# esq4/nind-denoise

Measured on AMD Instinct MI355X. Metric: megapixels/sec denoised, UtNet cs=256 on 24 MP frames, 1/2/4/8 MI355X, higher is better.
Workload: dtype f32; 1 GPU; configs[1]: one 6000x4000 (24.0 MP) fp32 frame per step, f32 storage in the conv stack (fp32 accumulate), UtNet(funit=64,PReLU) random-init (seed 123), cs=264 (nearest valid to the named size; the reference rejects 256 / 512) ucs=200 ol=64 -> 1276 tiles/frame, tiles per conv-stack launch 256, crop->infer->stitch device resident (frame and canvas in HBM); every tile's input is the whole cs x cs cro; tiles_per_frame=1276, parallelism=single GPU

## Files before the change

include/nind_hip.h:

```cpp
#ifndef NIND_HIP_H
#define NIND_HIP_H

#include <stddef.h>
#include <stdint.h>

#ifdef __cplusplus
extern "C" {
#endif

typedef enum nd_status {
    ND_OK = 0,
    ND_EINVAL = -1,
    ND_ENOMEM = -2,
    ND_EHIP = -3
} nd_status;

typedef enum nd_act {
    ND_ACT_NONE = 0,
    ND_ACT_PRELU = 1,
    ND_ACT_ELU = 2,
    ND_ACT_HARDSWISH = 3
} nd_act;

typedef enum nd_layer_kind {
    ND_CONV3 = 0,
    ND_CONVT3 = 1,
    ND_CONVT2S2 = 2,
    ND_CONV1 = 3,
    ND_CONV2S2 = 4
} nd_layer_kind;

typedef enum nd_dtype {
    ND_F32 = 0,
    ND_BF16 = 1,
    ND_F16 = 2
} nd_dtype;

typedef enum nd_flags {
    ND_FLAG_NO_SPLITK = 1,
    ND_FLAG_DIRECT_CONV = 2,
    ND_FLAG_W1D_REGS = 4,
    ND_FLAG_UNFUSED_POOL = 16,
    ND_FLAG_TILE_ENCODER = 32,
    ND_FLAG_TILE_LEVEL2 = 64,
    ND_FLAG_FIND_NOISE = 128,
    ND_FLAG_TILE_SKIPS = 256,
    ND_FLAG_TILE_WINO = 512,
    ND_FLAG_FULL_TILES = 8
} nd_flags;

int nd_version(void);
const char *nd_last_error(void);

int nd_tile_grid(int width, int height, int cs, int ucs, int ol, int *cols, int *rows, int *pad);
int nd_tile_geom(int i, int width, int height, int cs, int ucs, int ol,
                 int *x0, int *y0, int usefuldim[4], int usefulstart[2]);

int nd_tile_gather(const float *img_chw, int width, int height, int cs, int ucs, int ol,
                   int tile_begin, int tile_count, float *tiles_nchw, void *stream);
int nd_stitch_add(float *canvas_chw, int width, int height, int cs, int ucs, int ol,
                  const float *tiles_nchw, int tile_begin, int tile_count, void *stream);

int nd_utnet_num_tensors(void);
const char *nd_utnet_tensor_name(int idx);
size_t nd_utnet_packed_bytes(int funit, int dtype);
int nd_utnet_pack_weights(int funit, int dtype, const float *const *tensors, int n_tensors,
                          void *packed_host, size_t packed_bytes);

int nd_utnet_pack_weights_device(int funit, int dtype, const float *const *dev_tensors, int n_tensors, void *packed_dev,
                                 size_t packed_bytes, void *stream);
// ... 91 lines not shown
                               void *const *bucket_events, int n_events);
int nd_utnet_grad_buckets(int funit, size_t *offsets, size_t *counts, int max);
int nd_adam_step(float *params, const float *grads, float *m, float *v, float *vmax, size_t n, float lr, float beta1,
                 float beta2, float eps, int step, int amsgrad, void *stream);

size_t nd_ssim_workspace_bytes(int n, int c, int h, int w);
int nd_ssim(const float *x, const float *y, int n, int c, int h, int w, float *out, void *workspace, size_t workspace_bytes,
            void *stream);
int nd_ms_ssim(const float *x, const float *y, int n, int c, int h, int w, float *out, void *workspace,
               size_t workspace_bytes, void *stream);
int nd_mse(const float *x, const float *y, size_t count, float *out, void *workspace, size_t workspace_bytes, void *stream);

size_t nd_ssim_loss_workspace_bytes(int n, int c, int h, int w);
int nd_ssim_loss_grad(const float *x, const float *y, int n, int c, int h, int w, int multiscale, float weight,
                      float *loss_acc, float *gx, int accumulate, void *workspace, size_t workspace_bytes, void *stream);

size_t nd_ssim_padded_workspace_bytes(int n, int c, int h, int w, int window);
int nd_ssim_padded(const float *x, const float *y, int n, int c, int h, int w, int window, float *out, void *workspace,
                   size_t workspace_bytes, void *stream);
int nd_ssim_padded_grad(const float *x, const float *y, int n, int c, int h, int w, int window, const float *gout, float *gx,
                        void *workspace, size_t workspace_bytes, void *stream);

int nd_wino_mosaic(int p, int B, int *bx, int *by, long *tiles, long *tiles_per_image);

size_t nd_winograd_packed_bytes(int tile, int cin, int cout);
int nd_winograd_pack(int tile, int kind, int cin, int cout, const float *w, const float *bias, void *packed,
                     size_t packed_bytes);
size_t nd_layer_winograd_workspace_bytes(int tile, int kind, int batch, int cin, int cout, int h, int w);
int nd_layer_forward_winograd(int tile, int kind, int act, float slope, const void *packed, const float *x, int batch,
                              int cin, int h, int w, int cout, float *y, void *workspace, size_t workspace_bytes, int flags,
                              void *stream);

int nd_conv_bench(int kind, int dtype, int batch, int cin, int cout, int h, int w, int variant, int iters,
                  void *workspace, size_t workspace_bytes, void *stream, float *mean_ms);

int nd_winograd_bench(int tile, int kind, int batch, int cin, int cout, int h, int w, int iters, void *workspace,
                      size_t workspace_bytes, void *stream, float *mean_ms);
int nd_winograd_bench_flags(int tile, int kind, int batch, int cin, int cout, int h, int w, int iters, int flags, void *workspace,
                            size_t workspace_bytes, void *stream, float *mean_ms);

int nd_num_conv_variants(void);
const char *nd_conv_variant_name(int variant);

#ifdef __cplusplus
}
#endif
// ... 2 lines not shown
```

nind_denoise_amd/_lib.py:

```python
import ctypes
import os
from ctypes import POINTER, c_char_p, c_double, c_float, c_int, c_long, c_size_t, c_void_p

_HERE = os.path.dirname(os.path.abspath(__file__))
LIB_PATH = os.path.join(_HERE, "libnind_hip.so")

ND_F32, ND_BF16, ND_F16 = 0, 1, 2
DTYPE = {"f32": 0, "fp32": 0, "float32": 0, "bf16": 1, "bfloat16": 1, "f16": 2, "fp16": 2, "float16": 2}
ACT = {"none": 0, "PReLU": 1, "ELU": 2, "Hardswish": 3}
KIND = {"conv3": 0, "convT3": 1, "convT2s2": 2, "conv1": 3, "conv2s2": 4}
FLAG_NO_SPLITK, FLAG_DIRECT_CONV, FLAG_W1D_REGS, FLAG_FULL_TILES, FLAG_UNFUSED_POOL, FLAG_TILE_ENCODER, FLAG_TILE_LEVEL2 = 1, 2, 4, 8, 16, 32, 64
FLAG_FIND_NOISE = 128
FLAG_TILE_SKIPS = 256
FLAG_TILE_WINO = 512
PROGRESS_FN = ctypes.CFUNCTYPE(None, c_void_p, c_int, c_int, c_int)


class StepProfile(ctypes.Structure):
    _fields_ = [("ms", c_float), ("ms_xform_in", c_float), ("ms_gemm", c_float), ("ms_xform_out", c_float),
                ("form", c_int), ("kind", c_int), ("flops", c_double), ("mfma_flops", c_double), ("bytes", c_double),
                ("xform_bytes_in", c_double), ("xform_bytes_out", c_double)]


FORM_NAMES = {-1: "pool", 0: "direct", 1: "w1d_f43", 2: "w1d_f23", 3: "wino3p_f6x6"}


class NindHipError(RuntimeError):
    pass


class NindHipMissing(ImportError):
    pass


_lib = None

# ... 55 lines not shown
    "nd_utnet_train_workspace_bytes_hw": (c_size_t, [c_int] * 4),
    "nd_utnet_train_workspace_init_hw": (c_int, [c_void_p, c_size_t, c_int, c_int, c_int, c_int, c_void_p]),
    "nd_utnet_train_forward_hw": (c_int, [c_int, c_int, c_int, c_void_p, c_void_p, c_void_p, c_void_p, c_int, c_int, c_int, c_void_p,
                                          c_size_t, c_void_p]),
    "nd_utnet_train_backward_hw": (c_int, [c_int, c_int, c_int, c_void_p, c_void_p, c_void_p, c_void_p, c_void_p, c_int, c_int, c_int,
                                           c_void_p, c_size_t, c_void_p, POINTER(c_void_p), c_int]),
    "nd_utnet_train_step_hw": (c_int, [c_int, c_int, c_void_p, c_void_p, c_void_p, c_void_p, c_void_p, c_void_p, c_float, c_float,
                                       c_float, c_float, c_void_p, c_int, c_int, c_int, c_int, c_void_p, c_size_t, c_void_p,
                                       POINTER(c_void_p), c_int]),
    "nd_adam_step": (c_int, [c_void_p] * 5 + [c_size_t, c_float, c_float, c_float, c_float, c_int, c_int, c_void_p]),
    "nd_ssim_workspace_bytes": (c_size_t, [c_int] * 4),
    "nd_ssim": (c_int, [c_void_p, c_void_p] + [c_int] * 4 + [c_void_p, c_void_p, c_size_t, c_void_p]),
    "nd_ms_ssim": (c_int, [c_void_p, c_void_p] + [c_int] * 4 + [c_void_p, c_void_p, c_size_t, c_void_p]),
    "nd_ssim_loss_workspace_bytes": (c_size_t, [c_int] * 4),
    "nd_ssim_loss_grad": (c_int, [c_void_p, c_void_p] + [c_int] * 5 + [c_float, c_void_p, c_void_p, c_int, c_void_p, c_size_t,
                                  c_void_p]),
    "nd_ssim_padded_workspace_bytes": (c_size_t, [c_int] * 5),
    "nd_ssim_padded": (c_int, [c_void_p, c_void_p] + [c_int] * 5 + [c_void_p, c_void_p, c_size_t, c_void_p]),
    "nd_ssim_padded_grad": (c_int, [c_void_p, c_void_p] + [c_int] * 5 + [c_void_p, c_void_p, c_void_p, c_size_t, c_void_p]),
    "nd_mse": (c_int, [c_void_p, c_void_p, c_size_t, c_void_p, c_void_p, c_size_t, c_void_p]),
    "nd_conv_bench": (c_int, [c_int] * 9 + [c_void_p, c_size_t, c_void_p, POINTER(c_float)]),
    "nd_winograd_bench": (c_int, [c_int] * 8 + [c_void_p, c_size_t, c_void_p, POINTER(c_float)]),
    "nd_winograd_bench_flags": (c_int, [c_int] * 9 + [c_void_p, c_size_t, c_void_p, POINTER(c_float)]),
    "nd_wino_mosaic": (c_int, [c_int, c_int, POINTER(c_int), POINTER(c_int), POINTER(c_long), POINTER(c_long)]),
    "nd_num_conv_variants": (c_int, []),
    "nd_conv_variant_name": (c_char_p, [c_int]),
}

EXPORTS = tuple(_SIGNATURES)


def load():
    global _lib
    if _lib is not None:
        return _lib
    if not os.path.isfile(LIB_PATH):
        raise NindHipMissing(
            f"{LIB_PATH} not found: build it with `make -C nind_denoise_amd/csrc` (or __graft_entry__.build()). "
            "nind_denoise_amd has no CPU fallback for the denoise hot path.")
    import torch
    lib = ctypes.CDLL(LIB_PATH)
    for name, (res, args) in _SIGNATURES.items():
        fn = getattr(lib, name)
        fn.restype = res
        fn.argtypes = args
    _lib = lib
# ... 39 lines not shown
```

nind_denoise_amd/csrc/nd_common.h:

```cpp
#pragma once
#include <hip/hip_runtime.h>

#include <stdarg.h>
#include <stdint.h>
#include <stdio.h>

#include "nind_hip.h"

void nd_set_error(const char *fmt, ...);
#define ND_FAIL(code, ...)        \
    do {                          \
        nd_set_error(__VA_ARGS__); \
        return (code);            \
    } while (0)
#define ND_HIP(call)                                                                         \
    do {                                                                                     \
        hipError_t e_ = (call);                                                              \
        if (e_ != hipSuccess) ND_FAIL(ND_EHIP, "%s failed: %s", #call, hipGetErrorString(e_)); \
    } while (0)
#define ND_TRY(call)        \
    do {                    \
        int r_ = (call);    \
        if (r_ != 0) return r_; \
    } while (0)
// ... 9 lines not shown
    long np() const { return pstride; }
    long used() const { return (long)B * Hb * Wb; }
};

struct ConvDesc {
    int kind = ND_CONV3;
    int act = ND_ACT_NONE;
    float slope = 1.f;
    const float *slope_dev = nullptr;
    const float *wpk = nullptr;
    const float *bias = nullptr;
    int cin = 0, cout = 0;
    QpBuf in = {};
    QpBuf out = {};
    int out_plane0 = 0;
    int variant = -1;
    int in_plane0 = 0;
    float *pre = nullptr;
    long pre_plane = 0;
    float *part = nullptr;
    size_t part_bytes = 0;
    bool nosplit = false;
    bool tile_wino = false;
    int nbatch = 1;
    long in_bs = 0, out_bs = 0;
    size_t w_bs = 0;
    const QpBuf *pool = nullptr;
    int roi_r0 = 0, roi_c0 = 0, roi_rows = 0, roi_cols = 0;
    QpBuf in2 = {};
    int in2_plane0 = 0, in2_from = 0;
    const int *in2_origin = nullptr;
    long in2_origin_max = 0;
    int w_kb = 0, w_kb0 = 0;
    QpBuf add = {};
    int add_plane0 = 0;
    const int *add_origin = nullptr;
    long add_origin_max = 0;
};
int nd_check_in2(const char *who, const ConvDesc &d, int KB, long reach);
int nd_check_add(const char *who, const ConvDesc &d, long reach);
static const size_t kSplitScratchBytes = (size_t)512 * 64 * 1024 * 4;
int nd_launch_conv(const ConvDesc &d, hipStream_t stream);
bool nd_conv_pool_fits(const ConvDesc &d);
bool nd_conv_roi_fits(const ConvDesc &d);
int nd_conv_variant_count();
int nd_conv_variant_gemm(int cin, int cout);
// ... 2 lines not shown
size_t nd_wino_scratch_bytes(int T, const QpBuf &in, int cin, int cout);
int nd_launch_conv_wino(int T, const ConvDesc &d, void *scratch, size_t scratch_bytes, hipStream_t s, hipEvent_t *ev2 = nullptr);
long nd_wino_launch_tiles(int T, const ConvDesc &d);
void nd_wino_xform_bytes(int T, const QpBuf &in, int cin, int cout, long tiles, double *bytes_in, double *bytes_out);
size_t nd_w1d_packed_floats(int T, int cin, int cout);
int nd_w1d_pack(int T, int kind, int cin, int cout, const float *w, const float *bias, float *packed);
bool nd_w1d_fits(int T, const QpBuf &in);
int nd_launch_conv_w1d(int T, const ConvDesc &d, hipStream_t stream);
bool nd_w2d_ok(const QpBuf &in);
long nd_w2d_tiles(const QpBuf &in, int cout);
int nd_launch_conv_w2d(const ConvDesc &d, hipStream_t stream);
bool nd_f43_w2d(const QpBuf &in, int cout, bool pre, int flags);
int nd_launch_conv_f43(const ConvDesc &d, int flags, hipStream_t stream);
static inline size_t nd_buf_slack(int Wb) { return (size_t)10 * Wb + 8 + 2048; }
int nd_device(int *dev, int *ncus = nullptr);
int nd_raise_lds(int dev, const void *fn, size_t bytes);
int nd_once_per_device(int dev, int (*init)());
int nd_check_in_planes(const char *who, const ConvDesc &d, int KB, bool takes_in2 = false, bool takes_add = false);
int nd_check_out(const char *who, const ConvDesc &d, int oh, int ow, bool at_least);
int nd_check_int32(const char *who, const QpBuf &in);
int nd_check_roi(const char *who, const ConvDesc &d, int Hv, int Wv, bool refused, const char *why);
static inline int nd_check_flags(int flags, bool frame_loop = false, bool unet_frame = false) {
    const int known = ND_FLAG_NO_SPLITK | ND_FLAG_DIRECT_CONV | ND_FLAG_W1D_REGS | ND_FLAG_FULL_TILES | ND_FLAG_UNFUSED_POOL |
                      ND_FLAG_TILE_ENCODER | ND_FLAG_TILE_WINO | (frame_loop ? ND_FLAG_TILE_LEVEL2 | ND_FLAG_TILE_SKIPS : 0) | (unet_frame ? ND_FLAG_FIND_NOISE : 0);
    if (flags & ~known) ND_FAIL(ND_EINVAL, "unknown flag bits 0x%x", flags);
    return ND_OK;
}
const char *nd_conv_variant_label(int v);

static inline int nd_mtiles(int kind, int cout) {
    return kind == ND_CONVT2S2 ? (4 * cout + 255) / 256 * 8 : (cout + 127) / 128 * 4;
}
struct NdUpRow { int a, b, co; };
__host__ __device__ static inline NdUpRow nd_up_row(int m, int cout, int dt) {
    NdUpRow r;
    const int cpp = dt == ND_F32 ? 4 : 8, q = cout / cpp;
    const int G = m / (2 * cpp), e = m % cpp;
    r.b = (m / cpp) & 1;
    r.a = G / q;
    r.co = cpp * (G % q) + e;
    return r;
}
static inline int nd_taps(int kind) { return (kind == ND_CONV3 || kind == ND_CONVT3) ? 9 : (kind == ND_CONV2S2 ? 4 : 1); }
static inline int nd_kblocks(int cin, int dt = ND_F32) { return (cin + 2 * nd_cpp(dt) - 1) / (2 * nd_cpp(dt)); }
static inline size_t nd_bias_offset(int kind, int cin, int cout, int dt = ND_F32, int w1d_T = 0) {
    return (size_t)nd_mtiles(kind, cout) * nd_kblocks(cin, dt) * (w1d_T ? 3 * (w1d_T + 2) : nd_taps(kind)) * 256;
}
// ... 37 lines not shown
```

nind_denoise_amd/csrc/pack.hip:

```cpp
#include <string.h>

#include "nd_common.h"

static thread_local char g_err[512] = "";

void nd_set_error(const char *fmt, ...) {
    va_list ap;
    va_start(ap, fmt);
    vsnprintf(g_err, sizeof(g_err), fmt, ap);
    va_end(ap);
}

extern "C" const char *nd_last_error(void) { return g_err; }
extern "C" int nd_version(void) { return 112; }

static inline uint16_t f32_to_bf16_rne(float f) {
    uint32_t u;
    memcpy(&u, &f, 4);
    if ((u & 0x7fffffffu) > 0x7f800000u) return (uint16_t)((u >> 16) | 0x40);
    return (uint16_t)((u + 0x7fffu + ((u >> 16) & 1u)) >> 16);
}
static inline uint16_t f32_to_f16_rne(float f) {
    const _Float16 h = (_Float16)f;
    uint16_t u;
    memcpy(&u, &h, 2);
    return u;
}

void nd_pack_layer(int kind, int cin, int cout, int dt, const float *w, const float *bias, float *packed) {
    const int taps = nd_taps(kind);
    const int KB = nd_kblocks(cin, dt);
    const int MT = nd_mtiles(kind, cout);
    const int M = kind == ND_CONVT2S2 ? 4 * cout : cout;
    const int cpp = nd_cpp(dt);
    float *bp = packed + nd_bias_offset(kind, cin, cout, dt);
    auto weff = [&](int m, int ci, int t) -> float {
        if (m >= M || ci >= cin) return 0.f;
// ... 51 lines not shown
```

nind_denoise_amd/csrc/utnet.hip:

```cpp
#include <string.h>

#include <string>
#include <vector>

#include "nd_common.h"

#include "utnet_net.h"

extern "C" int nd_utnet_num_tensors(void) { return (int)tensor_names().size(); }
extern "C" const char *nd_utnet_tensor_name(int idx) {
    const auto &n = tensor_names();
    return (idx >= 0 && idx < (int)n.size()) ? n[idx].c_str() : nullptr;
}

extern "C" size_t nd_utnet_packed_bytes(int funit, int dtype) {
    if (check_funit(funit, dtype) != ND_OK) return 0;
    return blob_layout(funit, dtype).total * sizeof(float);
}

extern "C" int nd_utnet_pack_weights(int funit, int dtype, const float *const *tensors, int n_tensors, void *packed_host,
                                     size_t packed_bytes) {
    ND_TRY(check_funit(funit, dtype));
    if (n_tensors != nd_utnet_num_tensors()) ND_FAIL(ND_EINVAL, "nd_utnet_pack_weights: expected %d tensors, got %d", nd_utnet_num_tensors(), n_tensors);
    const BlobLayout bl = blob_layout(funit, dtype);
// ... 627 lines not shown
    d.part_bytes = kSplitScratchBytes;
    return d;
}
int launch_form(const LayerForm &fm, const ConvDesc &d, void *scratch, size_t scratch_bytes, hipStream_t s) {
    switch (fm.fam) {
        case LF_W1D: return nd_launch_conv_w1d(fm.T, d, s);
        case LF_W2D: return nd_launch_conv_w2d(d, s);
        case LF_WINO3P: return nd_launch_conv_wino(fm.T, d, scratch, scratch_bytes, s);
        default: return nd_launch_conv(d, s);
    }
}

int layer_forward(const LayerForm &fm, int kind, int act, float slope, int dt, const void *packed, const float *x, int batch,
                  int cin, int h, int w, int cout, float *y, void *ws, size_t ws_bytes, int variant, int flags, hipStream_t s) {
    const LayerPlan pl = layer_plan(kind, batch, cin, cout, h, w, (char *)ws, dt);
    ND_HIP(hipMemsetAsync(ws, 0, pl.bytes, s));
    ND_TRY(nd_launch_nchw_to_qp(x, cin, pl.in, 0, s));
    ConvDesc d = layer_desc(fm, kind, cin, cout, dt, (const float *)packed, pl);
    d.act = act;
    d.slope = slope;
    d.variant = variant;
    d.nosplit = (flags & ND_FLAG_NO_SPLITK) != 0;
    d.tile_wino = (flags & ND_FLAG_TILE_WINO) != 0;
    ND_TRY(launch_form(fm, d, (char *)ws + pl.bytes, ws_bytes - pl.bytes, s));
    return nd_launch_qp_to_nchw(pl.out, 0, y, cout, s);
}
}

extern "C" size_t nd_layer_workspace_bytes(int kind, int batch, int cin, int cout, int h, int w, int dtype) {
    if (dtype < ND_F32 || dtype > ND_F16 || kind < 0 || kind > 4 || batch <= 0 || cin <= 0 || cout <= 0 || h <= 0 || w <= 0) return 0;
    if (kind == ND_CONV3 && (h < 3 || w < 3)) return 0;
    return layer_plan(kind, batch, cin, cout, h, w, nullptr, dtype).bytes;
}

extern "C" int nd_layer_forward(int kind, int act, float slope, int dtype, const void *packed, const float *x, int batch,
                                int cin, int h, int w, int cout, float *y, void *ws, size_t ws_bytes, int variant, int flags,
                                void *stream) {
    ND_TRY(nd_check_flags(flags));
    if (dtype < ND_F32 || dtype > ND_F16) ND_FAIL(ND_EINVAL, "nd_layer_forward: unsupported dtype %d", dtype);
    const size_t need = nd_layer_workspace_bytes(kind, batch, cin, cout, h, w, dtype);
    if (!need) ND_FAIL(ND_EINVAL, "nd_layer_forward: bad shape");
    if (!ws || ws_bytes < need) ND_FAIL(ND_ENOMEM, "nd_layer_forward: workspace %zu B given, %zu B needed", ws_bytes, need);
    if (cout % nd_cpp(dtype)) ND_FAIL(ND_EINVAL, "nd_layer_forward: cout must be a multiple of %d", nd_cpp(dtype));
    return layer_forward(kDirect, kind, act, slope, dtype, packed, x, batch, cin, h, w, cout, y, ws, ws_bytes, variant, flags,
                         (hipStream_t)stream);
}
// ... 133 lines not shown

extern "C" int nd_winograd_bench(int tile, int kind, int batch, int cin, int cout, int h, int w, int iters, void *ws,
                                 size_t ws_bytes, void *stream, float *mean_ms) {
    return nd_winograd_bench_flags(tile, kind, batch, cin, cout, h, w, iters, 0, ws, ws_bytes, stream, mean_ms);
}
extern "C" int nd_winograd_bench_flags(int tile, int kind, int batch, int cin, int cout, int h, int w, int iters, int flags, void *ws,
                                       size_t ws_bytes, void *stream, float *mean_ms) {
    ND_TRY(nd_check_flags(flags));
    const size_t need = nd_layer_winograd_workspace_bytes(tile, kind, batch, cin, cout, h, w);
    if (!need) ND_FAIL(ND_EINVAL, "nd_winograd_bench: bad shape / kind / tile");
    const LayerForm fm = wino_form(tile);
    const size_t wfloats = wino_packed_floats(fm, cin, cout);
    const size_t total = ((need + 255) & ~(size_t)255) + wfloats * 4;
    if (!ws || ws_bytes < total) ND_FAIL(ND_ENOMEM, "nd_winograd_bench: workspace %zu B given, %zu B needed", ws_bytes, total);
    hipStream_t s = (hipStream_t)stream;
    LayerPlan pl = layer_plan(kind, batch, cin, cout, h, w, (char *)ws, ND_F32);
    float *wpk = (float *)((char *)ws + ((need + 255) & ~(size_t)255));
    fill_random(ws, pl.bytes, wpk, wfloats, ND_F32, kind, cin, cout, s);
    ConvDesc d = layer_desc(fm, kind, cin, cout, ND_F32, wpk, pl);
    d.act = ND_ACT_PRELU;
    d.slope = 0.2f;
    d.nosplit = (flags & ND_FLAG_NO_SPLITK) != 0;
    d.tile_wino = (flags & ND_FLAG_TILE_WINO) != 0;
    return time_form("nd_winograd_bench", fm, d, (char *)ws + pl.bytes, need - pl.bytes, iters, s, mean_ms);
}
```

nind_denoise_amd/csrc/utnet_net.h:

```cpp
#pragma once
#include <string.h>

#include <string>
#include <vector>

#include "nd_common.h"

namespace {

struct LayerSpec {
    const char *key;
    int kind;
    int cin_mul, cout_mul;
    int prelu;
};

const LayerSpec kLayers[] = {
    {"convs1.0", ND_CONV3, 0, 1, 0},    {"convs1.2", ND_CONV3, 1, 1, 1},    {"convs2.0", ND_CONV3, 1, 2, 2},
    {"convs2.2", ND_CONV3, 2, 2, 3},    {"convs3.0", ND_CONV3, 2, 4, 4},    {"convs3.2", ND_CONV3, 4, 4, 5},
    {"convs4.0", ND_CONV3, 4, 8, 6},    {"convs4.2", ND_CONV3, 8, 8, 7},    {"bottom.0", ND_CONV3, 8, 16, 8},
    {"bottom.2", ND_CONVT3, 16, 16, 9}, {"up1", ND_CONVT2S2, 16, 8, -1},    {"tconvs1.0", ND_CONVT3, 16, 8, 10},
    {"tconvs1.2", ND_CONVT3, 8, 8, 11}, {"up2", ND_CONVT2S2, 8, 4, -1},     {"tconvs2.0", ND_CONVT3, 8, 4, 12},
    {"tconvs2.2", ND_CONVT3, 4, 4, 13}, {"up3", ND_CONVT2S2, 4, 2, -1},     {"tconvs3.0", ND_CONVT3, 4, 2, 14},
    {"tconvs3.2", ND_CONVT3, 2, 2, 15}, {"up4", ND_CONVT2S2, 2, 1, -1},     {"tconvs4.0", ND_CONVT3, 2, 1, 16},
// ... 350 lines not shown
        }
        const LayerSpec &l = kLayers[st.layer];
        ConvDesc d;
        d.kind = l.kind;
        d.act = l.prelu >= 0 ? act : ND_ACT_NONE;
        d.slope = 0.25f;
        d.slope_dev = (l.prelu >= 0 && act == ND_ACT_PRELU) ? blob + l.prelu : nullptr;
        if (pre && l.prelu >= 0) {
            d.pre = pre[l.prelu].base;
            d.pre_plane = pre[l.prelu].np();
        }
        const int cin = lcin(l, f);
        d.cin = cin;
        d.cout = lcout(l, f);
        d.wpk = blob + bl.off[st.layer];
        d.bias = d.wpk + nd_bias_offset(l.kind, d.cin, d.cout, dt);
        d.in = pl.buf[st.src];
        d.out = pl.buf[st.dst];
        d.out_plane0 = st.dst_plane0_mul * f / cpp;
        d.part = pl.split;
        d.part_bytes = kSplitScratchBytes;
        d.nosplit = (flags & ND_FLAG_NO_SPLITK) != 0;
        d.tile_wino = (flags & ND_FLAG_TILE_WINO) != 0;
        const Form form = step_form(st, f, dt, flags, pl, bl, o.train_w1);
        if (o.rois && o.rois[this_step].rows > 0) {
            d.roi_r0 = o.rois[this_step].r0;
            d.roi_c0 = o.rois[this_step].c0;
            d.roi_rows = o.rois[this_step].rows;
            d.roi_cols = o.rois[this_step].cols;
        }
        for (int i = 0; i < o.nsrc2; ++i)
            if (o.src2[i].step == k && o.src2[i].addend) {
                d.add = o.src2[i].buf;
                d.add_plane0 = o.src2[i].plane0;
                d.add_origin = o.src2[i].origin;
                d.add_origin_max = o.src2[i].origin_max;
                d.w_kb = nd_kblocks(cin, dt);
                d.cin = o.src2[i].from * cpp;
            } else if (o.src2[i].step == k) {
                d.in2 = o.src2[i].buf;
                d.in2_plane0 = o.src2[i].plane0;
                d.in2_from = o.src2[i].from;
                d.in2_origin = o.src2[i].origin;
                d.in2_origin_max = o.src2[i].origin_max;
            }
        const bool next_is_pool = this_step + 1 < step_end && kSteps[this_step + 1].layer < 0;
// ... 251 lines not shown
    fp->bytes += fp->fold_wino_bytes;
}
inline int launch_skip_fold(int f, int flags, const float *blob, const BlobLayout &bl, int step, Form form, const QpBuf &cat, int planes,
                            const Roi &roi, int tstep, int nrows, int cols, float *split, char *wino, size_t wino_bytes, hipStream_t s) {
    const LayerSpec &l = kLayers[kSteps[step].layer];
    const int cin = lcin(l, f);
    ConvDesc d;
    d.kind = l.kind;
    d.act = ND_ACT_NONE;
    d.cin = planes * 4;
    d.cout = lcout(l, f);
    d.wpk = blob + bl.w1off[kSteps[step].layer];
    d.bias = d.wpk + nd_bias_offset(l.kind, cin, d.cout, ND_F32, kW1dTile);
    d.w_kb = nd_kblocks(cin);
    d.w_kb0 = planes / 2;
    d.in = cat;
    d.in_plane0 = planes;
    d.out = cat;
    d.out.pad = 1;
    d.out_plane0 = 0;
    d.part = split;
    d.part_bytes = split ? kSplitScratchBytes : 0;
    d.nosplit = (flags & ND_FLAG_NO_SPLITK) != 0;
    d.roi_r0 = roi.r0;
    d.roi_c0 = roi.c0;
    d.roi_rows = (nrows - 1) * tstep + roi.rows;
    d.roi_cols = (cols - 1) * tstep + roi.cols;
    if (form != FORM_WINO3P) return nd_launch_conv_w2d(d, s);
    d.wpk = blob + bl.woff[kSteps[step].layer];
    d.bias = nullptr;
    const int r_end = d.roi_r0 + d.roi_rows;
    for (int r0 = d.roi_r0; r0 < r_end; r0 += kFoldRows) {
        ConvDesc c = d;
        const int rows = r_end - r0 < kFoldRows ? r_end - r0 : kFoldRows;
        c.in.base = c.out.base = cat.base + (size_t)r0 * cat.Wb * 4;
        c.in.Hb = c.out.Hb = rows + 2;
        c.roi_r0 = 0;
        c.roi_rows = rows;
        ND_TRY(nd_launch_conv_wino(kWinoTile, c, wino, wino_bytes, s));
    }
    return ND_OK;
}

int frame_plan(int f, int dt, int flags, int W, int H, int cs, int ucs, int ol, int batch, FramePlan *fp) {
    *fp = FramePlan();
    ND_TRY(check_funit(f, dt));
// ... 63 lines not shown
```

nind_denoise_amd/csrc/winograd.hip:

```cpp
#include <stdlib.h>

#include <algorithm>
#include <atomic>
#include <thread>
#include <vector>

#include "nd_common.h"

typedef float f32x4 __attribute__((ext_vector_type(4)));

namespace {

__device__ __forceinline__ void tile_pos(long t, int TX, int TY, int &tx, int &ty, int &b) {
    const unsigned u = (unsigned)t, row = u / (unsigned)TX;
    tx = (int)(u - row * (unsigned)TX);
    b = (int)(row / (unsigned)TY);
    ty = (int)(row - (unsigned)b * (unsigned)TY);
}

template <int T> struct Wino;
template <> struct Wino<2> {
    static constexpr int A = 4;
    template <typename V> __host__ __device__ static void bt(const V *d, V *o) {
        o[0] = d[0] - d[2];
// ... 235 lines not shown
            for (int i = 0; i < A; ++i) d[i] = (okj && T * ty + i < Hb) ? src[(long)i * rs] : zero;
            Wino<T>::bt(d, o);
#pragma unroll
            for (int i = 0; i < A; ++i) sm[tl * RS + i * A + j] = o[i];
            }
        }
    }
    __syncthreads();
    {
        const int i = threadIdx.x / NTL, tl = threadIdx.x % NTL;
        const long t = t0 + tl;
        if (t < tiles) {
            f32x4 r[A], o[A];
#pragma unroll
            for (int j = 0; j < A; ++j) r[j] = sm[tl * RS + i * A + j];
            Wino<T>::bt(r, o);
            f32x4 *dst = v + (long)q * vnp + t;
#pragma unroll
            for (int j = 0; j < A; ++j) dst[(long)(i * A + j) * vbs] = o[j];
        }
    }
}

template <int T, int NTL, bool ADD = false, bool MOSAIC = false>
__global__ __launch_bounds__(NTL * (T + 2)) void k_wino_out2(const f32x4 *__restrict__ m, long mnp, long mbs, int B, int TY, int TX, int Hv,
                                                             int Wv, const float *__restrict__ bias, int act, float slope_imm,
                                                             const float *__restrict__ slope_dev, f32x4 *__restrict__ out, long onp,
                                                             int out_plane0, long out_img_stride, int Wo, int opad, f32x4 *__restrict__ pool, long pnp,
                                                             int Hp, int Wp, int ppad, const f32x4 *__restrict__ add = nullptr, long add_np = 0,
                                                             const int *__restrict__ origin_add = nullptr, int W_add = 0, int mp = 0,
                                                             int mbx = 0, int mby = 0) {
    static_assert(!(MOSAIC && ADD), "the mosaic form has no addend");
    constexpr int A = Wino<T>::A, RS = T * A + 1, NTH = NTL * A;
    __shared__ f32x4 sr[NTL * RS];
    __shared__ f32x4 so[T][NTL * T];
    const long tiles = MOSAIC ? (long)TY * TX : (long)B * TY * TX;
    const long t0 = (long)blockIdx.x * NTL;
    const int q = blockIdx.y;
    const f32x4 bv = ADD ? f32x4{0.f, 0.f, 0.f, 0.f} : *(const f32x4 *)(bias + 4 * q);
    const float slope = act == ND_ACT_NONE ? 1.f : (slope_dev ? *slope_dev : slope_imm);
    auto activate = [&](f32x4 y) {
#pragma unroll
        for (int e = 0; e < 4; ++e) {
            const float u = y[e];
            switch (act) {
                case ND_ACT_ELU: y[e] = u > 0.f ? u : expm1f(u); break;
// ... 87 lines not shown
    g.vnp = g.mnp = g.tiles;
    const long slack = 4096;
    g.vbs = (long)(2 * nd_kblocks(cin)) * g.vnp + slack;
    g.mbs = (long)((cout + 3) / 4) * g.mnp + slack;
    g.v_bytes = (size_t)positions(T) * g.vbs * 16;
    g.m_bytes = (size_t)positions(T) * g.mbs * 16;
}
WinoGeo wino_geo(int T, const QpBuf &in, int cin, int cout, int roi_rows = 0, int roi_cols = 0) {
    WinoGeo g;
    g.Hv = roi_rows > 0 ? roi_rows : in.Hb - 2;
    g.Wv = roi_rows > 0 ? roi_cols : in.Wb - 2;
    g.TY = (g.Hv + T - 1) / T;
    g.TX = (g.Wv + T - 1) / T;
    g.tiles = (long)in.B * g.TY * g.TX;
    wino_strides(T, cin, cout, g);
    return g;
}
bool wino_mosaic_rule(int T, const ConvDesc &d, int *bx, int *by, long *tiles) {
    if (T != 6 || d.kind != ND_CONVT3 || d.tile_wino || d.nosplit || d.roi_rows > 0 || d.pool || d.in2.base || d.add.base || d.pre) return false;
    if (d.in.Hb != d.in.Wb) return false;
    if (d.in.pad != 2) return false;
    long per_image;
    return nd_wino_mosaic(d.in.Hb - 2, d.in.B, bx, by, tiles, &per_image) == 1;
}
WinoGeo wino_geo_launch(int T, const ConvDesc &d) {
    WinoGeo g = wino_geo(T, d.in, d.cin, d.cout, d.roi_rows, d.roi_cols);
    int bx, by;
    long tiles;
    if (!wino_mosaic_rule(T, d, &bx, &by, &tiles)) return g;
    g.mp = g.Hv;
    g.mbx = bx;
    g.mby = by;
    g.TY = (by * g.mp + T - 1) / T;
    g.TX = (bx * g.mp + T - 1) / T;
    g.tiles = tiles;
    wino_strides(T, d.cin, d.cout, g);
    return g;
}
}

size_t nd_wino_packed_floats(int T, int cin, int cout) {
    return (size_t)positions(T) * gemm_floats(cin, cout) + (size_t)(cout + 3) / 4 * 4;
}

int nd_wino_pack(int T, int kind, int cin, int cout, const float *w, const float *bias, float *packed) {
    if (T != 2 && T != 4 && T != 6) ND_FAIL(ND_EINVAL, "winograd: tile must be 2, 4 or 6");
// ... 18 lines not shown
                    g[ky][kx] = kind == ND_CONV3 ? w[(((size_t)co * cin + ci) * 3 + ky) * 3 + kx]
                                                 : w[(((size_t)ci * cout + co) * 3 + (2 - ky)) * 3 + (2 - kx)];
            for (int kx = 0; kx < 3; ++kx) {
                double c[3] = {g[0][kx], g[1][kx], g[2][kx]}, o[8];
                if (T == 2) Wino<2>::g(c, o); else if (T == 4) Wino<4>::g(c, o); else Wino<6>::g(c, o);
                for (int i = 0; i < A; ++i) tmp[i][kx] = o[i];
            }
            for (int i = 0; i < A; ++i) {
                double o[8];
                if (T == 2) Wino<2>::g(tmp[i], o); else if (T == 4) Wino<4>::g(tmp[i], o); else Wino<6>::g(tmp[i], o);
                for (int j = 0; j < A; ++j) U[i][j] = o[j];
            }
            for (int i = 0; i < A; ++i)
                for (int j = 0; j < A; ++j) u[((size_t)(i * A + j) * cout + co) * cin + ci] = (float)U[i][j];
        }
    });
    const size_t gf = gemm_floats(cin, cout);
    parallel_for(P, [&](int p) { nd_pack_layer(ND_CONV1, cin, cout, ND_F32, u.data() + (size_t)p * cout * cin, nullptr, packed + p * gf); });
    float *b = packed + (size_t)P * gf;
    for (int co = 0; co < (cout + 3) / 4 * 4; ++co) b[co] = (bias && co < cout) ? bias[co] : 0.f;
    return ND_OK;
}

extern "C" int nd_wino_mosaic(int p, int B, int *bx, int *by, long *tiles, long *tiles_per_image) {
    if (p <= 0 || B <= 0 || !bx || !by || !tiles || !tiles_per_image) ND_FAIL(ND_EINVAL, "nd_wino_mosaic: bad arguments");
    const long T = 6, per = (long)B * ((p + T - 1) / T) * ((p + T - 1) / T);
    *tiles_per_image = *tiles = per;
    *bx = *by = 0;
    if (p < 8 || B < 2) return 0;
    auto count = [&](int x) { return (((long)x * p + T - 1) / T) * (((long)((B + x - 1) / x) * p + T - 1) / T); };
    long fewest = count(1);
    for (int x = 2; x <= B; ++x) fewest = std::min(fewest, count(x));
    long best = -1;
    int best_x = 0, best_y = 0, best_skew = 0;
    for (int x = B; x >= 1; --x) {
        const int y = (B + x - 1) / x, skew = x > y ? x - y : y - x;
        const long n = count(x);
        if (n * 100 > fewest * 101) continue;
        if (best < 0 || skew < best_skew || (skew == best_skew && n < best)) {
            best = n;
            best_x = x;
            best_y = y;
            best_skew = skew;
        }
    }
    if (best * 10 > per * 9) return 0;
// ... 37 lines not shown
    const bool src2 = d.in2.base != nullptr;
    if (src2) {
        if (T != 6) ND_FAIL(ND_EINVAL, "winograd: only the F(6x6) form has a second input source");
        ND_TRY(nd_check_in2("winograd", d, nd_kblocks(d.cin), (long)(d.roi_r0 + g.Hv + 1) * d.in2.Wb + d.roi_c0 + g.Wv + 2));
    }
    if (add) ND_TRY(nd_check_add("winograd", d, (long)(d.roi_r0 + g.Hv - 1 + d.add.pad) * d.add.Wb + d.roi_c0 + g.Wv - 1 + d.add.pad + 1));
    ND_TRY(nd_check_out("winograd", d, d.in.Hb - 2, d.in.Wb - 2, false));
    const long roi_in = roi ? (long)d.roi_r0 * d.in.Wb + d.roi_c0 : 0, roi_out = roi ? (long)d.roi_r0 * d.out.Wb + d.roi_c0 : 0;
    const int vHb = g.Hv + 2, vWb = g.Wv + 2;
    const size_t need = nd_wino_scratch_bytes(T, d.in, d.cin, d.cout);
    if (!scratch || scratch_bytes < need) ND_FAIL(ND_ENOMEM, "winograd: scratch %zu B given, %zu B needed", scratch_bytes, need);
    if (mosaic) {
        const size_t mneed = ((g.v_bytes + 255) & ~(size_t)255) + ((g.m_bytes + 255) & ~(size_t)255);
        if (g.mp < 8 || g.mp != d.in.Wb - 2 || (long)g.mbx * g.mby < d.in.B || (long)g.TY * g.TX != g.tiles || mneed > need)
            ND_FAIL(ND_EINVAL, "winograd: mosaic %d x %d at pitch %d does not fit %d images / the scratch bound", g.mbx, g.mby, g.mp, d.in.B);
    }
    if (g.tiles >= (1L << 31)) ND_FAIL(ND_EINVAL, "winograd: %ld tiles exceed the 32-bit tile index", g.tiles);
    const int P = positions(T);
    f32x4 *v = (f32x4 *)scratch;
    f32x4 *m = (f32x4 *)((char *)scratch + ((g.v_bytes + 255) & ~(size_t)255));
    const int in_planes = 2 * nd_kblocks(d.cin), out_planes = d.cout / 4;
    const f32x4 *x = (const f32x4 *)d.in.base + (long)d.in_plane0 * d.in.np() + roi_in;
    dim3 gi((unsigned)((g.tiles + 255) / 256), in_planes);
    constexpr int kNtl = 16;
    dim3 gi2((unsigned)((g.tiles + kNtl - 1) / kNtl), in_planes);
    if (T == 2)
        hipLaunchKernelGGL(k_wino_input<2>, gi, dim3(256), 0, s, x, d.in.np(), d.in.Hb, d.in.Wb, d.in.B, g.TY, g.TX, v, g.vnp, g.vbs);
    else if (mosaic)
        hipLaunchKernelGGL((k_wino_in2<6, kNtl, true>), gi2, dim3(kNtl * 8), 0, s, x, d.in.np(), vHb, vWb, (long)d.in.Hb * d.in.Wb, d.in.Wb, d.in.B, g.TY, g.TX, v, g.vnp,
                           g.vbs, nullptr, 0L, 0, nullptr, in_planes, g.mp, g.mbx, g.mby);
    else if (T == 6)
        hipLaunchKernelGGL((k_wino_in2<6, kNtl>), gi2, dim3(kNtl * 8), 0, s, x, d.in.np(), vHb, vWb, (long)d.in.Hb * d.in.Wb, d.in.Wb, d.in.B, g.TY, g.TX, v, g.vnp, g.vbs,
                           src2 ? (const f32x4 *)d.in2.base + (long)d.in2_plane0 * d.in2.np() + (roi ? (long)d.roi_r0 * d.in2.Wb + d.roi_c0 : 0) : nullptr,
                           d.in2.np(), d.in2.Wb, d.in2_origin, src2 ? d.in2_from : in_planes);
    else
        hipLaunchKernelGGL(k_wino_input<4>, gi, dim3(256), 0, s, x, d.in.np(), d.in.Hb, d.in.Wb, d.in.B, g.TY, g.TX, v, g.vnp, g.vbs);
    ND_HIP(hipGetLastError());
    if (ev2) ND_HIP(hipEventRecord(ev2[0], s));

    ConvDesc e;
    e.kind = ND_CONV1;
    e.cin = d.cin;
    e.cout = d.cout;
    e.wpk = d.wpk;
    e.bias = d.wpk + nd_bias_offset(ND_CONV1, cin_w, d.cout);
    e.w_kb = d.w_kb;
    e.w_kb0 = d.w_kb0;
    e.in = {(float *)v, in_planes, gB, g.TY, g.TX, 0, g.vnp, ND_F32};
    e.out = {(float *)m, out_planes, gB, g.TY, g.TX, 0, g.mnp, ND_F32};
// ... 58 lines not shown
```

nind_denoise_amd/networks/UtNet.py:

```python
import ctypes

import torch
from torch import nn

from .. import _lib
from ..synth import utnet_layer_table, utnet_prelu_keys

_ACTIVATIONS = {"PReLU": nn.PReLU, "ELU": nn.ELU, "Hardswish": nn.Hardswish}
_SHORT_DTYPE = {_lib.ND_F32: "f32", _lib.ND_BF16: "bf16", _lib.ND_F16: "f16"}


def canonical_compute_dtype(name):
    if name not in _lib.DTYPE:
        raise ValueError(f"unknown compute dtype {name!r}; choose one of {', '.join(_lib.DTYPE)}")
    return _SHORT_DTYPE[_lib.DTYPE[name]]


def valid_cs(cs):
    return cs >= 104 and (cs - 56) % 16 == 0


def nearest_valid_cs(cs):
    k = (cs - 56 + 8) // 16
    return max(104, 16 * k + 56)
# ... 61 lines not shown
        if st.generation != ctx.generation:
            raise RuntimeError("UtNet backward: another forward of this module ran under autograd since this graph was built; its "
                               "activations are gone (one forward/backward in flight per module -- as the reference's training loop runs)")
        batch, h, w = ctx.geom
        want_dx, want_p = ctx.needs_input_grad[2], ctx.needs_input_grad[3:]
        gy = gy.to(torch.float32).contiguous()
        dx = torch.empty(batch, 3, h, w, dtype=torch.float32, device=gy.device) if want_dx else None
        with torch.cuda.device(gy.device):
            _lib.check(_lib.load().nd_utnet_train_backward_hw(model.funit, _lib.ACT[model.activation], model.flags,
                                                              st.flat.data_ptr(), st.grads.data_ptr() if any(want_p) else None,
                                                              st.blobs.data_ptr(), gy.data_ptr(), dx.data_ptr() if want_dx else None,
                                                              batch, h, w, st.ws.data_ptr(), st.ws.numel(), _lib.stream_ptr(gy.device),
                                                              None, 0), "nd_utnet_train_backward_hw")
        grads = []
        for n, shape, want in zip(ctx.names, ctx.shapes, want_p):
            off, cnt = st.ranges[n]
            grads.append(st.grads[off:off + cnt].view(shape).clone() if want else None)
        return (None, None, dx) + tuple(grads)


class UtNet(nn.Module):
    split_k = True
    mosaic_wino = True
    winograd = True
    w1d_regs = False
    useful_only = True
    fused_pool = True
    share_encoder = True
    share_level2 = True
    fold_skips = True

    def __init__(self, funit=64, activation='PReLU', compute_dtype='f32'):
        super().__init__()
        funit = int(funit)
        compute_dtype = canonical_compute_dtype(compute_dtype)
        if activation not in _ACTIVATIONS:
            exit(f'UtNet: unknown activation function: {activation}')
        self.funit, self.activation = funit, activation
        groups = {}
        for key, kind, cin, cout, k in utnet_layer_table(funit):
            if kind == "conv":
                layer = nn.Conv2d(cin, cout, k)
            elif kind == "convT":
                layer = nn.ConvTranspose2d(cin, cout, k)
            else:
                layer = nn.ConvTranspose2d(cin, cout, k, stride=2)
# ... 11 lines not shown
        for name in order:
            g = groups[name]
            self.add_module(name, nn.Sequential(*[g[i] for i in sorted(g)]) if isinstance(g, dict) else g)
        self._packed = {}
        self.pack_on_device = True
        self._workspaces = {}
        self.max_cached_workspaces = 2
        self.compute_dtype = compute_dtype
        self.weights_generation = 0

    def set_compute_dtype(self, name):
        self.compute_dtype = canonical_compute_dtype(name)
        return self

    @property
    def _dt(self):
        return _lib.DTYPE[self.compute_dtype]

    @property
    def flags(self):
        return ((0 if self.split_k else _lib.FLAG_NO_SPLITK) | (0 if self.winograd else _lib.FLAG_DIRECT_CONV) |
                (_lib.FLAG_W1D_REGS if self.w1d_regs else 0) | (0 if self.useful_only else _lib.FLAG_FULL_TILES) |
                (0 if self.fused_pool else _lib.FLAG_UNFUSED_POOL) | (0 if self.share_encoder else _lib.FLAG_TILE_ENCODER) |
                (0 if self.mosaic_wino else _lib.FLAG_TILE_WINO))

    @property
    def frame_flags(self):
        return self.flags | (0 if self.share_level2 else _lib.FLAG_TILE_LEVEL2) | (0 if self.fold_skips else _lib.FLAG_TILE_SKIPS)

    def _weights_key(self, device):
        return (str(device), self.weights_generation) + tuple((p.data_ptr(), p._version) for p in self.parameters())

    def packed_weights(self, device):
        key = self._weights_key(device)
        hit = self._packed.get(self.compute_dtype)
        if hit is not None and hit[0] == key:
            return hit[1]
        lib = _lib.load()
        sd = self.state_dict()
        names = _lib.utnet_tensor_names()
        nbytes = lib.nd_utnet_packed_bytes(self.funit, self._dt)
        if nbytes == 0:
            raise ValueError(f"UtNet: funit={self.funit} is not supported by the HIP path for {self.compute_dtype} "
                             "(multiple of 8 for f32, of 16 for bf16 / f16)")
        on_device = self.pack_on_device
        where = device if on_device else "cpu"
        keep = []
# ... 91 lines not shown
```

Before: 90.08 MP/s.

## Add row-walking Winograd F(6,3) input transform reusing overlapping rows

Adds a new Winograd input-transform kernel in which each workgroup walks down a few tile rows. It keeps the two overlapping input rows in registers between consecutive tile rows, so they are not reloaded from memory. The kernel is enabled by default for T=6, and a flag is added to opt out. It also zero-masks padding lines for convT3 layers. The cost is fewer workgroups and extra synchronisation per row, and the grid-size heuristic falls back to the old kernel when parallelism would be too low.

```diff
diff --git a/include/nind_hip.h b/include/nind_hip.h
--- a/include/nind_hip.h
+++ b/include/nind_hip.h
@@ -46,6 +46,7 @@
     ND_FLAG_FIND_NOISE = 128,
     ND_FLAG_TILE_SKIPS = 256,
     ND_FLAG_TILE_WINO = 512,
+    ND_FLAG_TILE_WINO_IN = 1024,
     ND_FLAG_FULL_TILES = 8
 } nd_flags;
 
@@ -183,6 +184,7 @@
                         void *workspace, size_t workspace_bytes, void *stream);
 
 int nd_wino_mosaic(int p, int B, int *bx, int *by, long *tiles, long *tiles_per_image);
+int nd_wino_in_rows(int TX, int TY, long images);
 
 size_t nd_winograd_packed_bytes(int tile, int cin, int cout);
 int nd_winograd_pack(int tile, int kind, int cin, int cout, const float *w, const float *bias, void *packed,
diff --git a/nind_denoise_amd/_lib.py b/nind_denoise_amd/_lib.py
--- a/nind_denoise_amd/_lib.py
+++ b/nind_denoise_amd/_lib.py
@@ -12,6 +12,7 @@
 FLAG_NO_SPLITK, FLAG_DIRECT_CONV, FLAG_W1D_REGS, FLAG_FULL_TILES, FLAG_UNFUSED_POOL, FLAG_TILE_ENCODER, FLAG_TILE_LEVEL2 = 1, 2, 4, 8, 16, 32, 64
 FLAG_FIND_NOISE = 128
 FLAG_TILE_SKIPS = 256
+FLAG_TILE_WINO_IN = 1024
 FLAG_TILE_WINO = 512
 PROGRESS_FN = ctypes.CFUNCTYPE(None, c_void_p, c_int, c_int, c_int)
 
@@ -113,6 +114,7 @@
     "nd_conv_bench": (c_int, [c_int] * 9 + [c_void_p, c_size_t, c_void_p, POINTER(c_float)]),
     "nd_winograd_bench": (c_int, [c_int] * 8 + [c_void_p, c_size_t, c_void_p, POINTER(c_float)]),
     "nd_winograd_bench_flags": (c_int, [c_int] * 9 + [c_void_p, c_size_t, c_void_p, POINTER(c_float)]),
+    "nd_wino_in_rows": (c_int, [c_int, c_int, c_long]),
     "nd_wino_mosaic": (c_int, [c_int, c_int, POINTER(c_int), POINTER(c_int), POINTER(c_long), POINTER(c_long)]),
     "nd_num_conv_variants": (c_int, []),
     "nd_conv_variant_name": (c_char_p, [c_int]),
diff --git a/nind_denoise_amd/csrc/nd_common.h b/nind_denoise_amd/csrc/nd_common.h
--- a/nind_denoise_amd/csrc/nd_common.h
+++ b/nind_denoise_amd/csrc/nd_common.h
@@ -55,6 +55,7 @@
     size_t part_bytes = 0;
     bool nosplit = false;
     bool tile_wino = false;
+    bool tile_wino_in = false;
     int nbatch = 1;
     long in_bs = 0, out_bs = 0;
     size_t w_bs = 0;
@@ -103,7 +104,7 @@
 int nd_check_roi(const char *who, const ConvDesc &d, int Hv, int Wv, bool refused, const char *why);
 static inline int nd_check_flags(int flags, bool frame_loop = false, bool unet_frame = false) {
     const int known = ND_FLAG_NO_SPLITK | ND_FLAG_DIRECT_CONV | ND_FLAG_W1D_REGS | ND_FLAG_FULL_TILES | ND_FLAG_UNFUSED_POOL |
-                      ND_FLAG_TILE_ENCODER | ND_FLAG_TILE_WINO | (frame_loop ? ND_FLAG_TILE_LEVEL2 | ND_FLAG_TILE_SKIPS : 0) | (unet_frame ? ND_FLAG_FIND_NOISE : 0);
+                      ND_FLAG_TILE_ENCODER | ND_FLAG_TILE_WINO | ND_FLAG_TILE_WINO_IN | (frame_loop ? ND_FLAG_TILE_LEVEL2 | ND_FLAG_TILE_SKIPS : 0) | (unet_frame ? ND_FLAG_FIND_NOISE : 0);
     if (flags & ~known) ND_FAIL(ND_EINVAL, "unknown flag bits 0x%x", flags);
     return ND_OK;
 }
diff --git a/nind_denoise_amd/csrc/pack.hip b/nind_denoise_amd/csrc/pack.hip
--- a/nind_denoise_amd/csrc/pack.hip
+++ b/nind_denoise_amd/csrc/pack.hip
@@ -12,7 +12,7 @@
 }
 
 extern "C" const char *nd_last_error(void) { return g_err; }
-extern "C" int nd_version(void) { return 112; }
+extern "C" int nd_version(void) { return 113; }
 
 static inline uint16_t f32_to_bf16_rne(float f) {
     uint32_t u;
diff --git a/nind_denoise_amd/csrc/utnet.hip b/nind_denoise_amd/csrc/utnet.hip
--- a/nind_denoise_amd/csrc/utnet.hip
+++ b/nind_denoise_amd/csrc/utnet.hip
@@ -673,6 +673,7 @@
     d.variant = variant;
     d.nosplit = (flags & ND_FLAG_NO_SPLITK) != 0;
     d.tile_wino = (flags & ND_FLAG_TILE_WINO) != 0;
+    d.tile_wino_in = (flags & ND_FLAG_TILE_WINO_IN) != 0;
     ND_TRY(launch_form(fm, d, (char *)ws + pl.bytes, ws_bytes - pl.bytes, s));
     return nd_launch_qp_to_nchw(pl.out, 0, y, cout, s);
 }
@@ -852,5 +853,6 @@
     d.slope = 0.2f;
     d.nosplit = (flags & ND_FLAG_NO_SPLITK) != 0;
     d.tile_wino = (flags & ND_FLAG_TILE_WINO) != 0;
+    d.tile_wino_in = (flags & ND_FLAG_TILE_WINO_IN) != 0;
     return time_form("nd_winograd_bench", fm, d, (char *)ws + pl.bytes, need - pl.bytes, iters, s, mean_ms);
 }
diff --git a/nind_denoise_amd/csrc/utnet_net.h b/nind_denoise_amd/csrc/utnet_net.h
--- a/nind_denoise_amd/csrc/utnet_net.h
+++ b/nind_denoise_amd/csrc/utnet_net.h
@@ -396,6 +396,7 @@
         d.part_bytes = kSplitScratchBytes;
         d.nosplit = (flags & ND_FLAG_NO_SPLITK) != 0;
         d.tile_wino = (flags & ND_FLAG_TILE_WINO) != 0;
+        d.tile_wino_in = (flags & ND_FLAG_TILE_WINO_IN) != 0;
         const Form form = step_form(st, f, dt, flags, pl, bl, o.train_w1);
         if (o.rois && o.rois[this_step].rows > 0) {
             d.roi_r0 = o.rois[this_step].r0;
@@ -693,6 +694,7 @@
     d.part = split;
     d.part_bytes = split ? kSplitScratchBytes : 0;
     d.nosplit = (flags & ND_FLAG_NO_SPLITK) != 0;
+    d.tile_wino_in = (flags & ND_FLAG_TILE_WINO_IN) != 0;
     d.roi_r0 = roi.r0;
     d.roi_c0 = roi.c0;
     d.roi_rows = (nrows - 1) * tstep + roi.rows;
diff --git a/nind_denoise_amd/csrc/winograd.hip b/nind_denoise_amd/csrc/winograd.hip
--- a/nind_denoise_amd/csrc/winograd.hip
+++ b/nind_denoise_amd/csrc/winograd.hip
@@ -1,3 +1,4 @@
+#include <limits.h>
 #include <stdlib.h>
 
 #include <algorithm>
@@ -281,6 +282,77 @@
     }
 }
 
+template <int T, int NTL, bool MOSAIC = false>
+__global__ __launch_bounds__(NTL * (T + 2)) void k_wino_in2_rows(const f32x4 *__restrict__ x, long xnp, int Hb, int Wb, long img_stride, int row_stride,
+                                                                 int B, int TY, int TX, f32x4 *__restrict__ v, long vnp, long vbs,
+                                                                 const f32x4 *__restrict__ x2, long x2np, int row_stride2,
+                                                                 const int *__restrict__ origin2, int q2, int rows, int y_lo, int y_hi,
+                                                                 int mp = 0, int mbx = 0, int mby = 0) {
+    constexpr int A = Wino<T>::A, RS = A * A + 1;
+    __shared__ f32x4 sm[NTL * RS];
+    const int q = blockIdx.y;
+    const f32x4 zero = {0.f, 0.f, 0.f, 0.f};
+    const unsigned NRY = (unsigned)(TY + rows - 1) / (unsigned)rows, walks = (MOSAIC ? 1u : (unsigned)B) * NRY;
+    const unsigned bid = blockIdx.x, g = bid / walks, walk = bid - g * walks, b = MOSAIC ? 0u : walk / NRY, ry = walk - b * NRY;
+    const int ty0 = (int)ry * rows, nrow = min(rows, TY - ty0);
+    const int tl = threadIdx.x / A, j = threadIdx.x % A, i2 = threadIdx.x / NTL, tl2 = min((int)threadIdx.x % NTL, TX - 1 - (int)g * NTL);
+    const int tx = (int)g * NTL + tl, X = T * tx + j;
+    int y = T * ty0, cy = 0;
+    bool col_ok = tx < TX && X < Wb, img_ok = true;
+    const f32x4 *p;
+    long rs, wrap = 0;
+    if constexpr (MOSAIC) {
+        const unsigned cx = (unsigned)X / (unsigned)mp, lx = (unsigned)X - cx * (unsigned)mp;
+        cy = (int)((unsigned)y / (unsigned)mp);
+        y -= cy * mp;
+        rs = row_stride;
+        wrap = (long)mbx * img_stride - (long)mp * rs;
+        col_ok = tx < TX && (int)cx < mbx;
+        p = x + (long)q * xnp + ((long)cy * mbx + cx) * img_stride + (long)y * rs + lx;
+        img_ok = cy < mby && (long)cy * mbx + cx < B;
+    } else {
+        const bool s2 = q >= q2;
+        rs = s2 ? row_stride2 : row_stride;
+        p = (s2 ? x2 + (long)(q - q2) * x2np + origin2[b] : x + (long)q * xnp + (long)b * img_stride) + (long)y * rs + X;
+    }
+    f32x4 d[A], o[A];
+    auto load = [&](int i) {
+        d[i] = (col_ok && img_ok && y < Hb && y >= y_lo && y <= y_hi) ? *p : zero;
+        ++y;
+        p += rs;
+        if constexpr (MOSAIC) {
+            if (y == mp) {
+                y = 0;
+                ++cy;
+                p += wrap;
+                img_ok = cy < mby && (long)cy * mbx + (long)((unsigned)X / (unsigned)mp) < B;
+            }
+        }
+    };
+#pragma unroll
+    for (int i = 0; i < A; ++i) load(i);
+    f32x4 *dst = v + (long)q * vnp + ((long)b * TY + ty0) * TX + (int)g * NTL + tl2;
+    for (int r = 0; r < nrow; ++r, dst += TX) {
+        Wino<T>::bt(d, o);
+        if (r) __syncthreads();
+#pragma unroll
+        for (int i = 0; i < A; ++i) sm[tl * RS + i * A + j] = o[i];
+        d[0] = d[T];
+        d[1] = d[T + 1];
+        if (r + 1 < nrow) {
+#pragma unroll
+            for (int i = 2; i < A; ++i) load(i);
+        }
+        __syncthreads();
+        f32x4 rr[A], oo[A];
+#pragma unroll
+        for (int jj = 0; jj < A; ++jj) rr[jj] = sm[tl2 * RS + i2 * A + jj];
+        Wino<T>::bt(rr, oo);
+#pragma unroll
+        for (int jj = 0; jj < A; ++jj) dst[(long)(i2 * A + jj) * vbs] = oo[jj];
+    }
+}
+
 template <int T, int NTL, bool ADD = false, bool MOSAIC = false>
 __global__ __launch_bounds__(NTL * (T + 2)) void k_wino_out2(const f32x4 *__restrict__ m, long mnp, long mbs, int B, int TY, int TX, int Hv,
                                                              int Wv, const float *__restrict__ bias, int act, float slope_imm,
@@ -414,6 +486,20 @@
     if (d.in.pad != 2) return false;
     long per_image;
     return nd_wino_mosaic(d.in.Hb - 2, d.in.B, bx, by, tiles, &per_image) == 1;
+}
+constexpr int kInNtl = 16, kInRows = 2;
+int wino_in_rows_rule(int TX, int TY, long images) {
+    if (TX < kInNtl || TY < 1 || images < 1) return 0;
+    int rmax = kInRows;
+#ifdef ND_WINO_IN_SWEEP
+    if (const char *e = getenv("ND_WINO_IN_ROWS")) rmax = atoi(e);
+    if (rmax <= 0) return 0;
+#endif
+    const long groups = (TX + kInNtl - 1) / kInNtl;
+    if (groups * kInNtl - TX > TX / 6) return 0;
+    while (rmax > 1 && images * ((TY + rmax - 1) / rmax) * groups < 8) rmax /= 2;
+    const int walks = (TY + rmax - 1) / rmax;
+    return (TY + walks - 1) / walks;
 }
 WinoGeo wino_geo_launch(int T, const ConvDesc &d) {
     WinoGeo g = wino_geo(T, d.in, d.cin, d.cout, d.roi_rows, d.roi_cols);
@@ -478,6 +564,8 @@
     return ND_OK;
 }
 
+extern "C" int nd_wino_in_rows(int TX, int TY, long images) { return wino_in_rows_rule(TX, TY, images); }
+
 extern "C" int nd_wino_mosaic(int p, int B, int *bx, int *by, long *tiles, long *tiles_per_image) {
     if (p <= 0 || B <= 0 || !bx || !by || !tiles || !tiles_per_image) ND_FAIL(ND_EINVAL, "nd_wino_mosaic: bad arguments");
     const long T = 6, per = (long)B * ((p + T - 1) / T) * ((p + T - 1) / T);
@@ -561,9 +649,24 @@
     const int in_planes = 2 * nd_kblocks(d.cin), out_planes = d.cout / 4;
     const f32x4 *x = (const f32x4 *)d.in.base + (long)d.in_plane0 * d.in.np() + roi_in;
     dim3 gi((unsigned)((g.tiles + 255) / 256), in_planes);
-    constexpr int kNtl = 16;
+    constexpr int kNtl = kInNtl;
     dim3 gi2((unsigned)((g.tiles + kNtl - 1) / kNtl), in_planes);
-    if (T == 2)
+    const int in_rows = T == 6 && !d.tile_wino_in ? wino_in_rows_rule(g.TX, g.TY, gB) : 0;
+    if (in_rows) {
+        const bool zero_lines = d.kind == ND_CONVT3 && d.in.pad == 2 && !roi && !src2 && !add;
+        const int y_lo = zero_lines ? 2 : 0, y_hi = zero_lines && !mosaic ? d.in.Hb - 3 : INT_MAX;
+        const long walks = (long)gB * ((g.TY + in_rows - 1) / in_rows), blocks = walks * ((g.TX + kNtl - 1) / kNtl);
+        if (blocks >= (1L << 31)) ND_FAIL(ND_EINVAL, "winograd: %ld workgroups of the input transform exceed the grid", blocks);
+        dim3 gr((unsigned)blocks, in_planes);
+        if (mosaic)
+            hipLaunchKernelGGL((k_wino_in2_rows<6, kNtl, true>), gr, dim3(kNtl * 8), 0, s, x, d.in.np(), vHb, vWb, (long)d.in.Hb * d.in.Wb, d.in.Wb, d.in.B, g.TY,
+                               g.TX, v, g.vnp, g.vbs, nullptr, 0L, 0, nullptr, in_planes, in_rows, y_lo, y_hi, g.mp, g.mbx, g.mby);
+        else
+            hipLaunchKernelGGL((k_wino_in2_rows<6, kNtl>), gr, dim3(kNtl * 8), 0, s, x, d.in.np(), vHb, vWb, (long)d.in.Hb * d.in.Wb, d.in.Wb, d.in.B, g.TY,
+                               g.TX, v, g.vnp, g.vbs,
+                               src2 ? (const f32x4 *)d.in2.base + (long)d.in2_plane0 * d.in2.np() + (roi ? (long)d.roi_r0 * d.in2.Wb + d.roi_c0 : 0) : nullptr,
+                               d.in2.np(), d.in2.Wb, d.in2_origin, src2 ? d.in2_from : in_planes, in_rows, y_lo, y_hi);
+    } else if (T == 2)
         hipLaunchKernelGGL(k_wino_input<2>, gi, dim3(256), 0, s, x, d.in.np(), d.in.Hb, d.in.Wb, d.in.B, g.TY, g.TX, v, g.vnp, g.vbs);
     else if (mosaic)
         hipLaunchKernelGGL((k_wino_in2<6, kNtl, true>), gi2, dim3(kNtl * 8), 0, s, x, d.in.np(), vHb, vWb, (long)d.in.Hb * d.in.Wb, d.in.Wb, d.in.B, g.TY, g.TX, v, g.vnp,
diff --git a/nind_denoise_amd/networks/UtNet.py b/nind_denoise_amd/networks/UtNet.py
--- a/nind_denoise_amd/networks/UtNet.py
+++ b/nind_denoise_amd/networks/UtNet.py
@@ -107,6 +107,7 @@
 class UtNet(nn.Module):
     split_k = True
     mosaic_wino = True
+    row_walk_wino = True
     winograd = True
     w1d_regs = False
     useful_only = True
@@ -164,7 +165,7 @@
         return ((0 if self.split_k else _lib.FLAG_NO_SPLITK) | (0 if self.winograd else _lib.FLAG_DIRECT_CONV) |
                 (_lib.FLAG_W1D_REGS if self.w1d_regs else 0) | (0 if self.useful_only else _lib.FLAG_FULL_TILES) |
                 (0 if self.fused_pool else _lib.FLAG_UNFUSED_POOL) | (0 if self.share_encoder else _lib.FLAG_TILE_ENCODER) |
-                (0 if self.mosaic_wino else _lib.FLAG_TILE_WINO))
+                (0 if self.mosaic_wino else _lib.FLAG_TILE_WINO) | (0 if self.row_walk_wino else _lib.FLAG_TILE_WINO_IN))
 
     @property
     def frame_flags(self):
```

Measured after the change: 89.87 MP/s (median of 2 runs). About the same (-0.2%).
